# ndoll1998/lightgrad

Measured on AMD Instinct MI355X. Metric: mnist_mlp_train_steps_per_sec_batch1024_per_gpu, higher is better.
Workload: dtype f32; 1 GPU; mnist_mlp_784x512x10_bias_batch1024_mse_adabelief_lr1e-3 (fwd+bwd+allreduce+optimizer); batch_per_gpu=1024, global_batch=1024, parallelism=dp1, optimizer_kernel=fused, input_requires_grad=True, dispatch=hipGraph replay (python tape captured once; 13 consecutive steps per graph), steps_per_graph=13, device=AMD Instinct (gfx950), compute_units=256, clock_mhz=2400

## Files before the change

lightgrad_amd/csrc/gemm.hip:

```cpp
#include "common.h"
#include "gelu_common.h"
#include "adam_common.h"
#include "tail_jobs.h"
#include "mse_finalize.h"
#include "head_fwd_body.h"
#include <cstdlib>
#include <type_traits>

namespace lg {

typedef float f32x16 __attribute__((ext_vector_type(16)));
typedef unsigned int u32x4 __attribute__((ext_vector_type(4)));
typedef float f32x4 __attribute__((ext_vector_type(4)));

#ifndef LG_SMALL_PD
#define LG_SMALL_PD 2
#endif
constexpr int kSmallTilePrefetch = LG_SMALL_PD;

struct FastDiv {
    uint32_t m, s;
    __device__ __forceinline__ int div(int n) const { return int((uint64_t(uint32_t(n)) * m) >> s); }
};
static FastDiv make_fastdiv(int64_t d) {
    if (d < 1) d = 1;
    uint32_t l = 0;
    while ((int64_t(1) << l) < d) ++l;
    FastDiv f;
    f.m = uint32_t((uint64_t(1) << (31 + l)) / uint64_t(d) + 1);
    f.s = 31 + l;
    return f;
}

struct GemmArgs {
    const float* A;
    const float* B;
    float*       C;
    int64_t M, N, K;
    int64_t lda, ldb, ldc;
    int64_t sA, sB, sC;
    int64_t sA2, sB2, sC2;
    int     batch_inner;
    int     tiles_m, tiles_n;
    int     nwg;
    int     accumulate;
    const float* bias;
    const float* addend;
    int64_t      ldadd;
    int     group_m;
    int     k_slices;
    int64_t k_per_slice;
    float*  W;
    int*    tickets;
    float*  rowsum;
    int     rowsum_accumulate;
    FastDiv div_per_batch, div_slices, div_gspan, div_group, div_last_group, div_batch_inner;
    int     k_tail;
    short   relu_a, relu_b;
    int     act;
    float*  aux;
    int     multi;
    int64_t boff[3], coff[3], biasoff[3];
    int     seg_k, seg_steps;
    int64_t seg_jump[2];
    const AdamPlan* adam_c;
    const AdamPlan* adam_r;
#ifdef LG_GEMM_TIMELINE
    unsigned long long* tl;
#endif
};

#ifdef LG_GEMM_TIMELINE
#define LG_TL(slot) do { if (g.tl && threadIdx.x == 0) g.tl[size_t(blockIdx.x) * 8 + (slot)] = wall_clock64(); } while (0)
#else
#define LG_TL(slot) do { } while (0)
#endif

__device__ __forceinline__ int xcd_remap(int bid, int nwg) {
    const int q = nwg >> 3, r = nwg & 7;
    const int xcd = bid & 7, pos = bid >> 3;
    const int base = xcd < r ? xcd * (q + 1) : r * (q + 1) + (xcd - r) * q;
    return base + pos;
}

template <int BM, int BN> constexpr bool kHasExtras = BM * BN < 256 * 256;
template <int BM, int BN, int KG = 1> constexpr bool kCanSplitK = kHasExtras<BM, BN> && KG == 1;
template <int BM, int BN, int KG = 1> constexpr bool kCanAdam = BM * BN <= 128 * 128 && KG == 1;

#ifdef LG_GEMM_GATHER_STAGING
template <int BM, int BN, bool XKC> constexpr bool kGatherStaging = !XKC && BM * BN == 256 * 256;
#else
template <int BM, int BN, bool XKC> constexpr bool kGatherStaging = false;
#endif
template <int BM, int BN, int BK, bool AKC, bool BKC, int KG>
constexpr int gemm_lds_floats() {
    constexpr int BKS = BK * KG;
    constexpr bool ALK = AKC || kGatherStaging<BM, BN, AKC>, BLK = BKC || kGatherStaging<BM, BN, BKC>;
    return 2 * ((ALK ? BM * (BKS + 4) : BKS * BM) + (BLK ? BN * (BKS + 4) : BKS * BN));
}

template <int BM, int BN, int BK, int WM, int WN, bool AKC, bool BKC, bool VA, bool VB, int PD, int KG = 1, int XT = 0>
__global__ void __launch_bounds__(WM * WN * KG * 64) sgemm_mfma(GemmArgs g) {
#define LG_TILE_OWNS_LDS 1
#define LG_TILE_BID blockIdx.x
#include "gemm_tile_body.inc"
#undef LG_TILE_OWNS_LDS
#undef LG_TILE_BID
}

struct HeadChain {
    HeadFwd h;
    int*    tickets;
    int     stride;
    int     per_row;
    int*    status;
};
static const HeadChain*& pending_chain() { static const HeadChain* p = nullptr; return p; }
constexpr int kChainTicketBase = 16384, kChainTicketStride = 32, kChainRowBlocks = 64;
template <int OMAX, int PD>
__global__ void __launch_bounds__(256) sgemm_bias_head_fwd(GemmArgs g, HeadChain c) {
    constexpr int BM = 64, BN = 32, BK = 32, WM = 2, WN = 1, KG = 2, XT = 0;
    constexpr bool AKC = true, BKC = true, VA = true, VB = true;
    __shared__ __attribute__((aligned(16))) float lds[gemm_lds_floats<BM, BN, BK, AKC, BKC, KG>()];
    if (int(blockIdx.x) < g.nwg) {
        int* const signal_tickets = c.tickets;
        const int signal_stride = c.stride, signal_per_row = c.per_row;
#define LG_TILE_OWNS_LDS 0
#define LG_TILE_BID int(blockIdx.x)
#undef LG_TILE_SIGNAL
#define LG_TILE_SIGNAL 1
#include "gemm_tile_body.inc"
#undef LG_TILE_SIGNAL
#undef LG_TILE_BID
#undef LG_TILE_OWNS_LDS
    } else {
        const HeadFwd& a = c.h;
        const int tid = threadIdx.x, lane = tid & 63, wave = tid >> 6;
        const int wn = a.outs * a.hidden;
        for (int i = tid * 4; i < wn; i += 1024) *reinterpret_cast<float4*>(lds + i) = *reinterpret_cast<const float4*>(a.w + i);
        const int64_t row0 = int64_t(int(blockIdx.x) - g.nwg) * 4;
        int* const ticket = c.tickets + int(row0 / BM) * c.stride;
        const int64_t block_rows = a.rows - (row0 / BM) * BM < BM ? a.rows - (row0 / BM) * BM : BM;
        const int readers = int((block_rows + 3) / 4);
        int* const flag = ticket + 16;
        int* const done = ticket + 17;
        __shared__ int seen;
        if (tid == 0) {
            int ok = 1;
            const unsigned long long t0 = wall_clock64();
            while (__hip_atomic_load(flag, __ATOMIC_RELAXED, __HIP_MEMORY_SCOPE_AGENT) == 0) {
                __builtin_amdgcn_s_sleep(2);
                if (wall_clock64() - t0 > 200000000ull) {
                    __hip_atomic_fetch_or(c.status, LG_STATUS_HANDOFF_TIMEOUT, __ATOMIC_RELAXED, __HIP_MEMORY_SCOPE_SYSTEM);
                    ok = 0;
                    break;
                }
            }
            seen = ok;
        }
        __syncthreads();
        __builtin_amdgcn_fence(__ATOMIC_ACQUIRE, "wavefront");
        const int64_t row = row0 + wave;
        if (row < a.rows) head_fwd_row<OMAX, true>(a, lds, row, lane);
        if (tid == 0 && seen) {
            if (__hip_atomic_fetch_add(done, 1, __ATOMIC_RELAXED, __HIP_MEMORY_SCOPE_AGENT) == readers - 1) {
                __hip_atomic_store(done, 0, __ATOMIC_RELAXED, __HIP_MEMORY_SCOPE_AGENT);
                __hip_atomic_store(flag, 0, __ATOMIC_RELAXED, __HIP_MEMORY_SCOPE_AGENT);
            }
        }
    }
}

template <int PD, bool SECOND_BKC = false>
__global__ void __launch_bounds__(256) sgemm_pair_wgrad_xgrad(GemmArgs first, GemmArgs second) {
    constexpr int L1 = gemm_lds_floats<64, 64, 32, false, false, 1>(), L2 = gemm_lds_floats<64, 64, 32, true, SECOND_BKC, 1>();
    __shared__ __attribute__((aligned(16))) float lds[L1 > L2 ? L1 : L2];
    constexpr int BM = 64, BN = 64, BK = 32, WM = 2, WN = 2, KG = 1, XT = 0;
    constexpr bool VA = true, VB = true;
#define LG_TILE_OWNS_LDS 0
    if (int(blockIdx.x) < first.nwg) {
        constexpr bool AKC = false, BKC = false;
        const GemmArgs& g = first;
#define LG_TILE_BID int(blockIdx.x)
#include "gemm_tile_body.inc"
#undef LG_TILE_BID
    } else {
        constexpr bool AKC = true, BKC = SECOND_BKC;
        const GemmArgs& g = second;
#define LG_TILE_BID (int(blockIdx.x) - first.nwg)
#include "gemm_tile_body.inc"
#undef LG_TILE_BID
    }
#undef LG_TILE_OWNS_LDS
}

int lg_mse_finalize_job(const float* row_loss, int64_t rows, float inv_n, float* loss);
struct PairFirsts { GemmArgs w[2]; };
struct LossJob {
    const float* row_loss;
    float*       loss;
    int64_t      rows;
    float        inv_n;
};
template <int PD>
__global__ void __launch_bounds__(256) sgemm_triple_wgrad2_xgrad(PairFirsts firsts, GemmArgs second, LossJob job) {
    constexpr int L1 = gemm_lds_floats<64, 64, 32, false, false, 1>(), L2 = gemm_lds_floats<64, 64, 32, true, false, 1>();
    __shared__ __attribute__((aligned(16))) float lds[L1 > L2 ? L1 : L2];
    constexpr int BM = 64, BN = 64, BK = 32, WM = 2, WN = 2, KG = 1, XT = 0;
    constexpr bool VA = true, VB = true;
#define LG_TILE_OWNS_LDS 0
    const int n0w = firsts.w[0].nwg, n1w = firsts.w[1].nwg;
    if (int(blockIdx.x) < n0w + n1w) {
        constexpr bool AKC = false, BKC = false;
        const int which = int(blockIdx.x) >= n0w ? 1 : 0;
        const GemmArgs g = firsts.w[which];
#define LG_TILE_BID (int(blockIdx.x) - (which ? n0w : 0))
#include "gemm_tile_body.inc"
#undef LG_TILE_BID
    } else if (int(blockIdx.x) < n0w + n1w + second.nwg) {
        constexpr bool AKC = true, BKC = false;
        const GemmArgs& g = second;
#define LG_TILE_BID (int(blockIdx.x) - n0w - n1w)
#include "gemm_tile_body.inc"
#undef LG_TILE_BID
    } else {
        finalize_loss(job.row_loss, job.rows, job.inv_n, job.loss, lds);
    }
#undef LG_TILE_OWNS_LDS
}

constexpr int kGroupMax = 14;
struct GroupProduct {
    const float* A;
    const float* B;
    float*       C;
    float*       W;
    int*         tickets;
    float*       rowsum;
    int64_t      M, N, K, lda, ldb, ldc, k_per_slice;
    int          tiles_m, tiles_n, nwg, accumulate, group_m, k_slices, rowsum_accumulate, k_tail;
    FastDiv      div_per_batch, div_slices, div_gspan, div_group, div_last_group, div_batch_inner;
};
static GroupProduct pack_product(const GemmArgs& g) {
    return GroupProduct{g.A, g.B, g.C, g.W, g.tickets, g.rowsum, g.M, g.N, g.K, g.lda, g.ldb, g.ldc, g.k_per_slice,
                        g.tiles_m, g.tiles_n, g.nwg, g.accumulate, g.group_m, g.k_slices, g.rowsum_accumulate, g.k_tail,
                        g.div_per_batch, g.div_slices, g.div_gspan, g.div_group, g.div_last_group, g.div_batch_inner};
}
__device__ __forceinline__ GemmArgs unpack_product(const GroupProduct& p) {
    GemmArgs g{};
    g.A = p.A; g.B = p.B; g.C = p.C; g.W = p.W; g.tickets = p.tickets; g.rowsum = p.rowsum;
    g.M = p.M; g.N = p.N; g.K = p.K; g.lda = p.lda; g.ldb = p.ldb; g.ldc = p.ldc; g.k_per_slice = p.k_per_slice;
    g.tiles_m = p.tiles_m; g.tiles_n = p.tiles_n; g.nwg = p.nwg; g.accumulate = p.accumulate; g.group_m = p.group_m;
    g.k_slices = p.k_slices; g.rowsum_accumulate = p.rowsum_accumulate; g.k_tail = p.k_tail;
    g.div_per_batch = p.div_per_batch; g.div_slices = p.div_slices; g.div_gspan = p.div_gspan; g.div_group = p.div_group;
    g.div_last_group = p.div_last_group; g.div_batch_inner = p.div_batch_inner;
    g.batch_inner = 1;
    return g;
}

struct GemmGroup {
    GroupProduct p[kGroupMax];
    int      first[kGroupMax + 1];
    int      count;
    const float* cs_in;
    float*       cs_out;
    int64_t      cs_rows, cs_cols, cs_ld;
    int          cs_accumulate, cs_wgs;
    int          tail_wgs;
    TailGroup    tail;
};

static_assert(sizeof(GemmGroup) <= 4096, "the group travels as kernel arguments");

template <int PD>
__global__ void __launch_bounds__(256) sgemm_group_wgrad(GemmGroup grp) {
    __shared__ __attribute__((aligned(16))) float lds[gemm_lds_floats<64, 64, 32, false, false, 1>()];
    constexpr int BM = 64, BN = 64, BK = 32, WM = 2, WN = 2, KG = 1, XT = 0;
    constexpr bool VA = true, VB = true, AKC = false, BKC = false;
    if (int(blockIdx.x) < grp.cs_wgs) {
        const int q = threadIdx.x >> 6, cl = threadIdx.x & 63;
        const int64_t col = int64_t(blockIdx.x) * 64 + cl;
        const bool live = col < grp.cs_cols;
        const float* in = grp.cs_in + (live ? col : 0);
        float acc[8] = {0.f, 0.f, 0.f, 0.f, 0.f, 0.f, 0.f, 0.f};
        int64_t r = q;
        for (; r + 28 < grp.cs_rows; r += 32) {
#pragma unroll
            for (int e = 0; e < 8; ++e) acc[e] += in[(r + 4 * e) * grp.cs_ld];
        }
        for (; r < grp.cs_rows; r += 4) acc[0] += in[r * grp.cs_ld];
        lds[threadIdx.x] = ((acc[0] + acc[1]) + (acc[2] + acc[3])) + ((acc[4] + acc[5]) + (acc[6] + acc[7]));
        __syncthreads();
        if (q == 0 && live) {
            const float v = (lds[cl] + lds[64 + cl]) + (lds[128 + cl] + lds[192 + cl]);
            grp.cs_out[col] = grp.cs_accumulate ? grp.cs_out[col] + v : v;
        }
        return;
    }
    const int bid = int(blockIdx.x) - grp.cs_wgs;
    if (bid >= grp.first[grp.count]) {
        tail_group_body(grp.tail, bid - grp.first[grp.count]);
        return;
    }
    int which = 0;
    while (which + 1 < grp.count && bid >= grp.first[which + 1]) ++which;
    const GemmArgs g = unpack_product(grp.p[which]);
#define LG_TILE_OWNS_LDS 0
#define LG_TILE_BID (bid - grp.first[which])
#include "gemm_tile_body.inc"
#undef LG_TILE_BID
#undef LG_TILE_OWNS_LDS
}

template <int BM, int BN, int BK, int WM, int WN, bool AKC, bool BKC, int KG>
static void launch_layout(const GemmArgs& g, bool va, bool vb) {
    dim3 grid(g.nwg), block(WM * WN * KG * 64);
    hipStream_t s = rt().stream;
    constexpr int PD = (BM * BN <= 64 * 64) ? kSmallTilePrefetch : 2;
    static_assert(BM * BN < 256 * 256 || PD <= 2, "a third K-tile in flight does not fit the 256x256 tile's 128 registers: ring registers would spill while their loads are in flight");
    if constexpr (kHasExtras<BM, BN>) {
        if constexpr (AKC && BKC)  { if (g.multi) { hipLaunchKernelGGL((sgemm_mfma<BM, BN, BK, WM, WN, AKC, BKC, true, true, PD, KG, 1>), grid, block, 0, s, g); return; } }
        if constexpr (AKC && !BKC) { if (g.seg_k) { hipLaunchKernelGGL((sgemm_mfma<BM, BN, BK, WM, WN, AKC, BKC, true, true, PD, KG, 2>), grid, block, 0, s, g); return; } }
    }
    if constexpr (!kHasExtras<BM, BN>) {
        hipLaunchKernelGGL((sgemm_mfma<BM, BN, BK, WM, WN, AKC, BKC, true, true, PD, KG>), grid, block, 0, s, g);
        return;
    }
    if (va && vb)  hipLaunchKernelGGL((sgemm_mfma<BM, BN, BK, WM, WN, AKC, BKC, true, true, PD, KG>), grid, block, 0, s, g);
    else if (va)   hipLaunchKernelGGL((sgemm_mfma<BM, BN, BK, WM, WN, AKC, BKC, true, false, 1, KG>), grid, block, 0, s, g);
    else if (vb)   hipLaunchKernelGGL((sgemm_mfma<BM, BN, BK, WM, WN, AKC, BKC, false, true, 1, KG>), grid, block, 0, s, g);
    else           hipLaunchKernelGGL((sgemm_mfma<BM, BN, BK, WM, WN, AKC, BKC, false, false, 1, KG>), grid, block, 0, s, g);
}

#ifdef LG_GEMM_TIMELINE
static void lg_debug_timeline_state(unsigned long long* buf, int nwg, int slices, int tiles);
#endif
struct PairState {
    int      active = 0;
    int      count = 0;
    bool     second_bkc = false;
    GemmArgs args[3];
    bool     is_s[3] = {false, false, false};
    int64_t  batch[3] = {1, 1, 1};
    int64_t  tiles = 0;
    LossJob  job{};
};
static PairState& pair_state() { static PairState p; return p; }

static void pair_launch_single(const GemmArgs& g, bool is_s) {
    dim3 grid(g.nwg), block(256);
    constexpr int PD = kSmallTilePrefetch;
    if (!is_s) hipLaunchKernelGGL((sgemm_mfma<64, 64, 32, 2, 2, false, false, true, true, PD, 1>), grid, block, 0, rt().stream, g);
    else if (pair_state().second_bkc) hipLaunchKernelGGL((sgemm_mfma<64, 64, 32, 2, 2, true, true, true, true, PD, 1>), grid, block, 0, rt().stream, g);
    else           hipLaunchKernelGGL((sgemm_mfma<64, 64, 32, 2, 2, true, false, true, true, PD, 1>), grid, block, 0, rt().stream, g);
}

static int pair_retune(GemmArgs& g, int64_t others_nwg) {
    const int64_t tiles = int64_t(g.tiles_m) * g.tiles_n;
    static const char* pair_slices_env = getenv("LG_GEMM_PAIR_SLICES");
    if (pair_slices_env || g.nwg != tiles * g.k_slices || g.seg_k || tiles >= 256 || g.K < 128) return LG_OK;
    constexpr int BK = 32, BM = 64, BN = 64;
    const double cus = rt().compute_units > 0 ? rt().compute_units : 256;
    const int64_t k_tiles = (g.K + BK - 1) / BK;
    int64_t best_sl = g.k_slices;
    double best = 1e30;
    for (int64_t sl = 1; sl <= 64 && (sl == 1 || sl * 2 <= k_tiles); ++sl) {
        const double per_cu = double(tiles * sl + others_nwg) / cus;
        const double c = per_cu > 1.0 ? double(int64_t(per_cu + 0.999)) : 1.0;
        const double cost = double((k_tiles + sl - 1) / sl) * (c <= 1.0 ? 0.68 : 0.43 * c + 0.17) + (sl > 1 ? 1.8 + 0.85 * double(sl) : 0.0);
        if (cost < best) { best = cost; best_sl = sl; }
    }
    int64_t k_per_slice = ((g.K + best_sl - 1) / best_sl + BK - 1) / BK * BK;
    best_sl = (g.K + k_per_slice - 1) / k_per_slice;
    if (best_sl == g.k_slices) return LG_OK;
    if (g.W) { const int rc = lg_free(g.W); g.W = nullptr; if (rc != LG_OK) return rc; }
    g.k_per_slice = k_per_slice;
    g.k_slices = int(best_sl);
    g.nwg = int(tiles * best_sl);
    g.div_slices = make_fastdiv(best_sl);
    if (best_sl > 1) {
        const int rc = lg_malloc(reinterpret_cast<void**>(&g.W), size_t(tiles * best_sl) * BM * BN * sizeof(float));
        if (rc != LG_OK) return rc;
    }
    return LG_OK;
}

static int pair_flush(bool keep_collecting) {
    PairState& P = pair_state();
    int rc = LG_OK;
    bool job_done = false;
    if (P.count == 3) {
        rc = pair_retune(P.args[1], int64_t(P.args[0].nwg) + P.args[2].nwg);
        if (rc != LG_OK) { P.count = 0; return rc; }
        PairFirsts firsts;
        firsts.w[0] = P.args[0];
        firsts.w[1] = P.args[1];
        const int spare = P.job.loss ? 1 : 0;
        hipLaunchKernelGGL((sgemm_triple_wgrad2_xgrad<kSmallTilePrefetch>), dim3(P.args[0].nwg + P.args[1].nwg + P.args[2].nwg + spare), dim3(256), 0,
                           rt().stream, firsts, P.args[2], P.job);
        job_done = true;
    } else if (P.count == 2 && P.is_s[1]) {
        rc = pair_retune(P.args[0], P.args[1].nwg);
        if (rc != LG_OK) { P.count = 0; return rc; }
#ifdef LG_GEMM_TIMELINE
        if (P.args[0].tl) {
            (void)hipMemsetAsync(P.args[0].tl, 0, size_t(P.args[0].nwg + P.args[1].nwg) * 64, rt().stream);
            lg_debug_timeline_state(P.args[0].tl, P.args[0].nwg + P.args[1].nwg, P.args[0].k_slices * 100 + P.args[1].k_slices, P.args[0].nwg);
        }
#endif
        if (P.second_bkc)
            hipLaunchKernelGGL((sgemm_pair_wgrad_xgrad<kSmallTilePrefetch, true>), dim3(P.args[0].nwg + P.args[1].nwg), dim3(256), 0, rt().stream,
                               P.args[0], P.args[1]);
        else
            hipLaunchKernelGGL((sgemm_pair_wgrad_xgrad<kSmallTilePrefetch, false>), dim3(P.args[0].nwg + P.args[1].nwg), dim3(256), 0, rt().stream,
                               P.args[0], P.args[1]);
    } else {
        for (int i = 0; i < P.count; ++i) pair_launch_single(P.args[i], P.is_s[i]);
    }
    for (int i = 0; i < P.count; ++i)
        if (P.args[i].W) { const int r = lg_free(P.args[i].W); if (r != LG_OK) rc = r; }
    P.count = 0;
    P.tiles = 0;
    if (job_done) P.job = LossJob{};
    if (!keep_collecting && P.active) P.active = 2;
    return rc;
}

struct WriteSpan { uintptr_t lo, hi; };
static WriteSpan product_c_span(const GemmArgs& g, int64_t batch) {
    const int64_t outer = batch / g.batch_inner;
    int64_t lo = 0, hi = (g.M - 1) * g.ldc + g.N;
    const int64_t reach[2] = {(outer - 1) * g.sC, int64_t(g.batch_inner - 1) * g.sC2};
    for (int64_t r : reach) { if (r < 0) lo += r; else hi += r; }
    const uintptr_t base = reinterpret_cast<uintptr_t>(g.C);
    return WriteSpan{base + uintptr_t(lo * 4), base + uintptr_t(hi * 4)};
}
static bool spans_meet(WriteSpan a, WriteSpan b) { return a.lo < b.hi && b.lo < a.hi; }
static bool products_write_alike(const GemmArgs& a, int64_t batch_a, const GemmArgs& b, int64_t batch_b) {
    const WriteSpan none{0, 0};
    const WriteSpan ca = product_c_span(a, batch_a), cb = product_c_span(b, batch_b);
    const WriteSpan ra = a.rowsum ? WriteSpan{reinterpret_cast<uintptr_t>(a.rowsum), reinterpret_cast<uintptr_t>(a.rowsum + a.M)} : none;
    const WriteSpan rb = b.rowsum ? WriteSpan{reinterpret_cast<uintptr_t>(b.rowsum), reinterpret_cast<uintptr_t>(b.rowsum + b.M)} : none;
    return spans_meet(ca, cb) || spans_meet(ca, rb) || spans_meet(ra, cb) || spans_meet(ra, rb);
}

static bool pair_try_defer(GemmArgs& g, bool akc, bool bkc, bool va, bool vb, int64_t batch) {
    PairState& P = pair_state();
    if (P.active != 1) return false;
    const int slot = P.count;
    for (int i = 0; i < slot; ++i)
        if (products_write_alike(P.args[i], P.batch[i], g, batch)) return false;
    const bool f_form = !akc && !bkc, s_form = akc;
    bool fits = slot < 3 && va && vb && batch >= 1;
    if (slot == 0)      fits = fits && f_form;
    else if (slot == 1) fits = fits && !P.is_s[0] && (f_form || s_form);
    else                fits = fits && !P.is_s[1] && s_form && !bkc && batch == 1 && !g.relu_a && !g.relu_b;
    if (slot == 1 && f_form) fits = fits && batch == 1 && P.args[0].nwg == int64_t(P.args[0].tiles_m) * P.args[0].tiles_n * P.args[0].k_slices;
    const int64_t tiles = int64_t(g.tiles_m) * g.tiles_n * batch;
    if (!fits || P.tiles + tiles > rt().n_gemm_tickets) return false;
    g.tickets = rt().gemm_tickets + P.tiles;
    P.tiles += tiles;
    if (s_form) P.second_bkc = bkc;
    P.is_s[slot] = s_form;
    P.args[slot] = g;
    P.batch[slot] = batch;
    P.count = slot + 1;
    return true;
}

constexpr int kGroupTiles = 1024;
struct GroupState {
    int       active = 0;
// ... 577 lines not shown
```

lightgrad_amd/csrc/gemm_tile_body.inc:

```
#ifndef LG_TILE_SIGNAL
#define LG_TILE_SIGNAL 0
#endif
    constexpr int NT = WM * WN * KG * 64;
    constexpr int BKS = BK * KG;
    constexpr int TM = BM / WM / 32, TN = BN / WN / 32;
    static_assert(TM >= 1 && TN >= 1 && BK % 16 == 0 && (KG == 1 || KG == 2 || KG == 4), "tile config");
    constexpr bool AG = kGatherStaging<BM, BN, AKC>, BG = kGatherStaging<BM, BN, BKC>;
    static_assert((!AG || VA) && (!BG || VB), "gather staging replaces the float4 form");
    constexpr bool ALK = AKC || AG, BLK = BKC || BG;
    constexpr int A_PITCH = ALK ? BKS + 4 : BM;
    constexpr int B_PITCH = BLK ? BKS + 4 : BN;
    constexpr int A_TILE = ALK ? BM * A_PITCH : BKS * A_PITCH;
    constexpr int B_TILE = BLK ? BN * B_PITCH : BKS * B_PITCH;
    constexpr int A_ELEMS = BM * BKS / NT, B_ELEMS = BN * BKS / NT;
    static_assert(A_ELEMS % 4 == 0 && B_ELEMS % 4 == 0, "staging must divide into float4");

    static_assert(2 * (A_TILE + B_TILE) == gemm_lds_floats<BM, BN, BK, AKC, BKC, KG>(), "LDS size");
    static_assert(!(AG || BG) || TM * TN > 1, "gather staging: the multi-accumulator loop only");
#if LG_TILE_OWNS_LDS
    __shared__ __attribute__((aligned(16))) float lds[2 * (A_TILE + B_TILE)];
#endif
    constexpr int BUF = A_TILE + B_TILE;

    const int tid = threadIdx.x;
    const int lane = tid & 63, wave = tid >> 6;
    const int kg = wave / (WM * WN), wl = wave % (WM * WN);
    const int wm = wl / WN, wn = wl % WN;
    const int kofs = kg * BK;
    const int r = lane & 31, h = lane >> 5;
    LG_TL(0);

    const int id = xcd_remap(LG_TILE_BID, g.nwg);
    const int per_batch = g.tiles_m * g.tiles_n;
    const int bs = g.div_per_batch.div(id);
    const int batch = g.div_slices.div(bs), slice = bs - batch * g.k_slices;
    const int t = id - bs * per_batch;
    const int GROUP_M = g.group_m;
    const int gspan = GROUP_M * g.tiles_n;
    const int group = g.div_gspan.div(t);
    const int first_m = group * GROUP_M, in_group = t - group * gspan;
    const bool last_group = g.tiles_m - first_m < GROUP_M;
    const int gsize = last_group ? g.tiles_m - first_m : GROUP_M;
    const int tn = last_group ? g.div_last_group.div(in_group) : g.div_group.div(in_group);
    const int tm = first_m + (in_group - tn * gsize);
    const int64_t m0 = int64_t(tm) * BM, n0 = int64_t(tn) * BN;
    const int b_outer = g.div_batch_inner.div(batch), b_inner = batch - b_outer * g.batch_inner;
    const float* __restrict__ A = g.A + int64_t(b_outer) * g.sA + int64_t(b_inner) * g.sA2;
    const float* Bp = g.B + int64_t(b_outer) * g.sB + int64_t(b_inner) * g.sB2;
    float* Cp = g.C + int64_t(b_outer) * g.sC + int64_t(b_inner) * g.sC2;
    const float* biasp = g.bias;
    if constexpr (XT == 1) {
        {
            Bp += batch == 0 ? g.boff[0] : batch == 1 ? g.boff[1] : g.boff[2];
            Cp += batch == 0 ? g.coff[0] : batch == 1 ? g.coff[1] : g.coff[2];
            if (biasp) biasp += batch == 0 ? g.biasoff[0] : batch == 1 ? g.biasoff[1] : g.biasoff[2];
        }
    }
    const float* __restrict__ B = Bp;
    float* __restrict__ C = Cp;
    const int64_t ldc = g.ldc;
    const int accumulate = g.accumulate;
    const float* __restrict__ bias = biasp;
    const int64_t k_begin = int64_t(slice) * g.k_per_slice;
    const int64_t k_end = (k_begin + g.k_per_slice < g.K) ? k_begin + g.k_per_slice : g.K;
    const bool has_virtual = kHasExtras<BM, BN> && g.rowsum != nullptr && n0 <= g.N && g.N < n0 + BN;

    using StageA = std::conditional_t<VA, f32x4, float>;
    using StageB = std::conditional_t<VB, f32x4, float>;
    constexpr int A_CHUNKS = VA ? A_ELEMS / 4 : A_ELEMS, B_CHUNKS = VB ? B_ELEMS / 4 : B_ELEMS;
    constexpr int NL = (kGatherStaging<BM, BN, AKC> ? 4 : 1) * A_CHUNKS + (kGatherStaging<BM, BN, BKC> ? 4 : 1) * B_CHUNKS;
    static_assert((PD - 1) * NL + NL <= 63, "vmcnt is a 6-bit counter");
    StageA ra_ring[PD][A_CHUNKS];
    StageB rb_ring[PD][B_CHUNKS];
    [[maybe_unused]] float ga_ring[PD][AG ? A_CHUNKS : 1][4];
    [[maybe_unused]] float gb_ring[PD][BG ? B_CHUNKS : 1][4];

    constexpr unsigned OOB = 0x80000000u;
    constexpr int A_W = VA ? 4 : 1, B_W = VB ? 4 : 1;
    constexpr int A_DIV = AG ? BM : (AKC ? BKS : BM) / A_W, B_DIV = BG ? BN : (BKC ? BKS : BN) / B_W;
    static_assert(NT % A_DIV == 0 && NT % B_DIV == 0, "a thread's chunks must differ by whole rows");
    constexpr int A_STEP = NT / A_DIV, B_STEP = NT / B_DIV;
    const int a_q = tid / A_DIV, a_r = AG ? tid % A_DIV : (tid % A_DIV) * A_W;
    const int b_q = tid / B_DIV, b_r = BG ? tid % B_DIV : (tid % B_DIV) * B_W;
    auto kcA = [&](int i) { return AG ? 4 * (a_q + i * A_STEP) : (AKC ? a_r : a_q + i * A_STEP); };
    auto kcB = [&](int i) { return BG ? 4 * (b_q + i * B_STEP) : (BKC ? b_r : b_q + i * B_STEP); };
    const int a_lds0 = AG ? a_r * A_PITCH + 4 * a_q : a_q * A_PITCH + a_r, b_lds0 = BG ? b_r * B_PITCH + 4 * b_q : b_q * B_PITCH + b_r;
    constexpr int A_LDS_STEP = AG ? 4 * A_STEP : A_STEP * A_PITCH, B_LDS_STEP = BG ? 4 * B_STEP : B_STEP * B_PITCH;
    unsigned offA[A_CHUNKS], offB[B_CHUNKS];
    unsigned virt_mask = 0;
    int krem_ring[PD];
#pragma unroll
    for (int i = 0; i < A_CHUNKS; ++i) {
        const int row = AKC ? a_q + i * A_STEP : a_r, kk = kcA(i);
        const unsigned bytes = AKC ? (unsigned(row) * unsigned(g.lda) + unsigned(kk)) * 4u : (unsigned(kk) * unsigned(g.lda) + unsigned(row)) * 4u;
        offA[i] = (m0 + row < g.M) ? bytes : OOB;
    }
#pragma unroll
    for (int i = 0; i < B_CHUNKS; ++i) {
        const int col = BKC ? b_q + i * B_STEP : b_r, kk = kcB(i);
        const unsigned bytes = BKC ? (unsigned(col) * unsigned(g.ldb) + unsigned(kk)) * 4u : (unsigned(kk) * unsigned(g.ldb) + unsigned(col)) * 4u;
        offB[i] = (n0 + col < g.N) ? bytes : OOB;
        if (has_virtual && n0 + col == g.N) virt_mask |= 1u << i;
    }
    const float* const Atile0 = AKC ? A + m0 * g.lda : A + m0;
    const float* const Btile0 = BKC ? B + n0 * g.ldb : B + n0;

    auto descriptor = [](const float* base) {
        const unsigned long long p = reinterpret_cast<unsigned long long>(base);
        u32x4 d;
        d[0] = unsigned(p); d[1] = unsigned(p >> 32) & 0xffffu; d[2] = OOB; d[3] = 0x00020000u;
        return d;
    };
    const float* nextA = AKC ? Atile0 + k_begin : Atile0 + k_begin * g.lda;
    const float* nextB = BKC ? Btile0 + k_begin : Btile0 + k_begin * g.ldb;
    const int64_t stepA = AKC ? int64_t(BKS) : int64_t(BKS) * g.lda, stepB = BKC ? int64_t(BKS) : int64_t(BKS) * g.ldb;
    [[maybe_unused]] const unsigned gatherA = unsigned(g.lda) * 4u, gatherB = unsigned(g.ldb) * 4u;
    const int nkt = int((k_end - k_begin + BKS - 1) / BKS);
    const int last_krem = int(k_end - k_begin) - (nkt - 1) * BKS;
    int requested = 0;
    int seg_left = 0, seg_idx = 0;
    if constexpr (XT == 2) seg_left = g.seg_steps;
    auto load_tile = [&](int slot) {
        const int krem = requested == nkt - 1 ? last_krem : BKS;
        ++requested;
        krem_ring[slot] = krem;
        const u32x4 da = descriptor(nextA);
        const u32x4 db = descriptor(nextB);
        nextA += stepA;
        nextB += stepB;
        if constexpr (XT == 2) {
            if (--seg_left == 0) {
                nextB += seg_idx ? g.seg_jump[1] : g.seg_jump[0];
                seg_idx = 1;
                seg_left = g.seg_steps;
            }
        }
#pragma unroll
        for (int i = 0; i < A_CHUNKS; ++i) {
            if constexpr (AG) {
                if (krem == BKS) {
#pragma unroll
                    for (int e = 0; e < 4; ++e)
                        asm volatile("buffer_load_dword %0, %1, %2, %3 offen" : "=v"(ga_ring[slot][i][e]) : "v"(offA[i]), "s"(da), "s"(unsigned(e) * gatherA));
                } else {
#pragma unroll
                    for (int e = 0; e < 4; ++e) {
                        const unsigned off = kcA(i) + e < krem ? offA[i] : OOB;
                        asm volatile("buffer_load_dword %0, %1, %2, %3 offen" : "=v"(ga_ring[slot][i][e]) : "v"(off), "s"(da), "s"(unsigned(e) * gatherA));
                    }
                }
            } else {
                const unsigned off = kcA(i) < krem ? offA[i] : OOB;
                if constexpr (VA) asm volatile("buffer_load_dwordx4 %0, %1, %2, 0 offen" : "=v"(ra_ring[slot][i]) : "v"(off), "s"(da));
                else              asm volatile("buffer_load_dword %0, %1, %2, 0 offen" : "=v"(ra_ring[slot][i]) : "v"(off), "s"(da));
            }
        }
#pragma unroll
        for (int i = 0; i < B_CHUNKS; ++i) {
            if constexpr (BG) {
                if (krem == BKS) {
#pragma unroll
                    for (int e = 0; e < 4; ++e)
                        asm volatile("buffer_load_dword %0, %1, %2, %3 offen" : "=v"(gb_ring[slot][i][e]) : "v"(offB[i]), "s"(db), "s"(unsigned(e) * gatherB));
                } else {
#pragma unroll
                    for (int e = 0; e < 4; ++e) {
                        const unsigned off = kcB(i) + e < krem ? offB[i] : OOB;
                        asm volatile("buffer_load_dword %0, %1, %2, %3 offen" : "=v"(gb_ring[slot][i][e]) : "v"(off), "s"(db), "s"(unsigned(e) * gatherB));
                    }
                }
            } else {
                const unsigned off = kcB(i) < krem ? offB[i] : OOB;
                if constexpr (VB) asm volatile("buffer_load_dwordx4 %0, %1, %2, 0 offen" : "=v"(rb_ring[slot][i]) : "v"(off), "s"(db));
                else              asm volatile("buffer_load_dword %0, %1, %2, 0 offen" : "=v"(rb_ring[slot][i]) : "v"(off), "s"(db));
            }
        }
    };
    auto wait_tile = [&](int slot, int younger) {
        if (PD >= 3 && younger >= 2)      asm volatile("s_waitcnt vmcnt(%0)" :: "n"(PD >= 3 ? 2 * NL : 0) : "memory");
        else if (PD >= 2 && younger == 1) asm volatile("s_waitcnt vmcnt(%0)" :: "n"(PD >= 2 ? NL : 0) : "memory");
        else                              asm volatile("s_waitcnt vmcnt(0)" ::: "memory");
#pragma unroll
        for (int i = 0; i < A_CHUNKS; ++i) {
            if constexpr (AG) { asm volatile("" : "+v"(ga_ring[slot][i][0]), "+v"(ga_ring[slot][i][1]), "+v"(ga_ring[slot][i][2]), "+v"(ga_ring[slot][i][3])); }
            else              asm volatile("" : "+v"(ra_ring[slot][i]));
        }
#pragma unroll
        for (int i = 0; i < B_CHUNKS; ++i) {
            if constexpr (BG) { asm volatile("" : "+v"(gb_ring[slot][i][0]), "+v"(gb_ring[slot][i][1]), "+v"(gb_ring[slot][i][2]), "+v"(gb_ring[slot][i][3])); }
            else              asm volatile("" : "+v"(rb_ring[slot][i]));
        }
    };

    auto store_tile = [&](int buf, int slot) {
        float* a = lds + buf * BUF;
        float* b = lds + buf * BUF + A_TILE;
        if (g.k_tail && krem_ring[slot] < BKS) {
            asm volatile("; short K tail" ::: "memory");
            if constexpr (VA && AKC) {
#pragma unroll
                for (int i = 0; i < A_CHUNKS; ++i)
#pragma unroll
                    for (int e = 1; e < 4; ++e)
                        if (kcA(i) + e >= krem_ring[slot]) ra_ring[slot][i][e] = 0.f;
            }
            if constexpr (VB && BKC) {
#pragma unroll
                for (int i = 0; i < B_CHUNKS; ++i)
#pragma unroll
                    for (int e = 1; e < 4; ++e)
                        if (kcB(i) + e >= krem_ring[slot]) rb_ring[slot][i][e] = 0.f;
            }
        }
        if constexpr (kHasExtras<BM, BN>) if (g.relu_a) {
            asm volatile("; relu(A) on the way to LDS" ::: "memory");
#pragma unroll
            for (int i = 0; i < A_CHUNKS; ++i) {
                if constexpr (VA) {
#pragma unroll
                    for (int e = 0; e < 4; ++e) { const float x = ra_ring[slot][i][e]; ra_ring[slot][i][e] = (x != x) ? x : (x > 0.0f ? x : 0.0f); }
                } else {
                    const float x = ra_ring[slot][i]; ra_ring[slot][i] = (x != x) ? x : (x > 0.0f ? x : 0.0f);
                }
            }
        }
#pragma unroll
        for (int i = 0; i < A_CHUNKS; ++i) {
            if constexpr (AG)      *reinterpret_cast<f32x4*>(a + a_lds0 + i * A_LDS_STEP) = f32x4{ga_ring[slot][i][0], ga_ring[slot][i][1], ga_ring[slot][i][2], ga_ring[slot][i][3]};
            else if constexpr (VA) *reinterpret_cast<f32x4*>(a + a_lds0 + i * A_LDS_STEP) = ra_ring[slot][i];
            else                   a[a_lds0 + i * A_LDS_STEP] = ra_ring[slot][i];
        }
        if constexpr (kHasExtras<BM, BN>) if (g.relu_b) {
            asm volatile("; relu(B) on the way to LDS" ::: "memory");
#pragma unroll
            for (int i = 0; i < B_CHUNKS; ++i) {
                if constexpr (VB) {
#pragma unroll
                    for (int e = 0; e < 4; ++e) { const float x = rb_ring[slot][i][e]; rb_ring[slot][i][e] = (x != x) ? x : (x > 0.0f ? x : 0.0f); }
                } else {
                    const float x = rb_ring[slot][i]; rb_ring[slot][i] = (x != x) ? x : (x > 0.0f ? x : 0.0f);
                }
            }
        }
        if constexpr (kHasExtras<BM, BN>) if (has_virtual) {
#pragma unroll
            for (int i = 0; i < B_CHUNKS; ++i) {
                const bool virt = (virt_mask >> i) & 1u, kv = kcB(i) < krem_ring[slot];
                const float one = kv ? 1.0f : 0.0f;
                if constexpr (VB) {
                    if constexpr (BKC) {
                        if (virt) {
                            const int kr = krem_ring[slot] - kcB(i);
                            rb_ring[slot][i] = f32x4{kr > 0 ? 1.f : 0.f, kr > 1 ? 1.f : 0.f, kr > 2 ? 1.f : 0.f, kr > 3 ? 1.f : 0.f};
                        }
                    }
                    else               { if (virt) rb_ring[slot][i] = f32x4{one, 0.f, 0.f, 0.f}; }
                } else {
                    if (virt) rb_ring[slot][i] = one;
                }
            }
        }
#pragma unroll
        for (int i = 0; i < B_CHUNKS; ++i) {
            if constexpr (BG)      *reinterpret_cast<f32x4*>(b + b_lds0 + i * B_LDS_STEP) = f32x4{gb_ring[slot][i][0], gb_ring[slot][i][1], gb_ring[slot][i][2], gb_ring[slot][i][3]};
            else if constexpr (VB) *reinterpret_cast<f32x4*>(b + b_lds0 + i * B_LDS_STEP) = rb_ring[slot][i];
            else                   b[b_lds0 + i * B_LDS_STEP] = rb_ring[slot][i];
        }
    };

    f32x16 acc[TM][TN];
    [[maybe_unused]] float bias_ahead[TN];
    if constexpr (kHasExtras<BM, BN>) {
#pragma unroll
        for (int j = 0; j < TN; ++j) {
            const int64_t col = n0 + (wn * TN + j) * 32 + r;
            bias_ahead[j] = (bias && col < g.N) ? bias[col] : 0.f;
        }
    }
#pragma unroll
    for (int i = 0; i < TM; ++i)
#pragma unroll
        for (int j = 0; j < TN; ++j)
#pragma unroll
            for (int e = 0; e < 16; ++e) acc[i][j][e] = 0.f;

    auto compute_tile = [&](int buf, int kb_begin, int kb_end) {
        const float* a = lds + buf * BUF + (ALK ? (wm * TM * 32 + r) * A_PITCH + 4 * h + kofs : (4 * h + kofs) * A_PITCH + wm * TM * 32 + r);
        const float* b = lds + buf * BUF + A_TILE + (BLK ? (wn * TN * 32 + r) * B_PITCH + 4 * h + kofs : (4 * h + kofs) * B_PITCH + wn * TN * 32 + r);
#pragma unroll
        for (int kb = kb_begin; kb < kb_end; kb += 8) {
            float fa[TM][4], fb[TN][4];
#pragma unroll
            for (int i = 0; i < TM; ++i) {
                if constexpr (ALK) {
                    const float4 v = *reinterpret_cast<const float4*>(a + i * 32 * A_PITCH + kb);
                    fa[i][0] = v.x; fa[i][1] = v.y; fa[i][2] = v.z; fa[i][3] = v.w;
                } else {
#pragma unroll
                    for (int s = 0; s < 4; ++s) fa[i][s] = a[(kb + s) * A_PITCH + i * 32];
                }
            }
#pragma unroll
            for (int j = 0; j < TN; ++j) {
                if constexpr (BLK) {
                    const float4 v = *reinterpret_cast<const float4*>(b + j * 32 * B_PITCH + kb);
                    fb[j][0] = v.x; fb[j][1] = v.y; fb[j][2] = v.z; fb[j][3] = v.w;
                } else {
#pragma unroll
                    for (int s = 0; s < 4; ++s) fb[j][s] = b[(kb + s) * B_PITCH + j * 32];
                }
            }
#pragma unroll
            for (int s = 0; s < 4; ++s)
#pragma unroll
                for (int i = 0; i < TM; ++i)
#pragma unroll
                    for (int j = 0; j < TN; ++j)
                        acc[i][j] = __builtin_amdgcn_mfma_f32_32x32x2f32(fa[i][s], fb[j][s], acc[i][j], 0, 0, 0);
        }
    };

#pragma unroll
    for (int u = 0; u < PD; ++u)
        if (u < nkt) load_tile(u);
    {
        const int younger = nkt - 1 < PD - 1 ? nkt - 1 : PD - 1;
        wait_tile(0, younger);
    }
    store_tile(0, 0);
    __syncthreads();
    LG_TL(1);
    if constexpr (TM * TN == 1) {
        constexpr int HG = BK / 16;
        float fa[2][HG][4], fb[2][HG][4];
        auto read_half = [&](int buf, int half, int slot) {
            const float* a = lds + buf * BUF + (AKC ? (wm * 32 + r) * A_PITCH + 4 * h + kofs : (4 * h + kofs) * A_PITCH + wm * 32 + r);
            const float* b = lds + buf * BUF + A_TILE + (BKC ? (wn * 32 + r) * B_PITCH + 4 * h + kofs : (4 * h + kofs) * B_PITCH + wn * 32 + r);
#pragma unroll
            for (int q = 0; q < HG; ++q) {
                const int kb = half * (BK / 2) + q * 8;
                if constexpr (AKC) {
                    const float4 v = *reinterpret_cast<const float4*>(a + kb);
                    fa[slot][q][0] = v.x; fa[slot][q][1] = v.y; fa[slot][q][2] = v.z; fa[slot][q][3] = v.w;
                } else {
#pragma unroll
                    for (int e = 0; e < 4; ++e) fa[slot][q][e] = a[(kb + e) * A_PITCH];
                }
                if constexpr (BKC) {
                    const float4 v = *reinterpret_cast<const float4*>(b + kb);
                    fb[slot][q][0] = v.x; fb[slot][q][1] = v.y; fb[slot][q][2] = v.z; fb[slot][q][3] = v.w;
                } else {
#pragma unroll
                    for (int e = 0; e < 4; ++e) fb[slot][q][e] = b[(kb + e) * B_PITCH];
                }
            }
        };
        auto mfma_part = [&](int slot, int q0, int q1) {
#pragma unroll
            for (int q = q0; q < q1; ++q)
#pragma unroll
                for (int e = 0; e < 4; ++e)
                    acc[0][0] = __builtin_amdgcn_mfma_f32_32x32x2f32(fa[slot][q][e], fb[slot][q][e], acc[0][0], 0, 0, 0);
        };
        auto mfma_half = [&](int slot) { mfma_part(slot, 0, HG); };
        constexpr int HQ = HG > 1 ? HG / 2 : HG;
        read_half(0, 0, 0);
        for (int kt0 = 0; kt0 < nkt; kt0 += PD) {
#pragma unroll
            for (int u = 0; u < PD; ++u) {
                const int kt = kt0 + u;
                if (kt < nkt) {
                    const int cur = kt & 1;
                    if (PD == 1 && kt + 1 < nkt) load_tile(0);
                    read_half(cur, 1, 1);
                    mfma_part(0, 0, HQ);
                    __builtin_amdgcn_sched_barrier(0);
                    if (kt + 1 < nkt) {
                        int younger = nkt - (kt + 2);
                        if (younger > PD - 2) younger = PD - 2;
                        wait_tile((u + 1) % PD, PD == 1 ? 0 : (younger < 0 ? 0 : younger));
                        store_tile(cur ^ 1, (u + 1) % PD);
                    }
                    if (PD > 1 && kt + PD < nkt) load_tile(u);
                    __builtin_amdgcn_sched_barrier(0);
                    mfma_part(0, HQ, HG);
                    __syncthreads();
                    if (kt + 1 < nkt) read_half(cur ^ 1, 0, 0);
                    mfma_half(1);
                }
            }
        }
    } else {
        for (int kt0 = 0; kt0 < nkt; kt0 += PD) {
    #pragma unroll
            for (int u = 0; u < PD; ++u) {
                const int kt = kt0 + u;
                if (kt < nkt) {
                    const int cur = kt & 1;
                    if (PD == 1 && kt + 1 < nkt) load_tile(0);
                    compute_tile(cur, 0, BK / 2);
                    if (kt + 1 < nkt) {
                        int younger = nkt - (kt + 2);
                        if (younger > PD - 2) younger = PD - 2;
                        wait_tile((u + 1) % PD, PD == 1 ? 0 : (younger < 0 ? 0 : younger));
                        store_tile(cur ^ 1, (u + 1) % PD);
                    }
                    if (PD > 1 && kt + PD < nkt) load_tile(u);
                    compute_tile(cur, BK / 2, BK);
                    __syncthreads();
                }
            }
        }
    }

    LG_TL(2);
    if constexpr (KG > 1) {
        constexpr int GROUP_FLOATS = WM * WN * TM * TN * 16 * 64;
        static_assert((KG - 1) * GROUP_FLOATS <= 2 * (A_TILE + B_TILE), "the K-group exchange must fit the staging buffers");
        float* x = lds + (wl * TM * TN * 16) * 64 + lane;
        if (kg >= 1) {
#pragma unroll
            for (int i = 0; i < TM; ++i)
#pragma unroll
                for (int j = 0; j < TN; ++j)
#pragma unroll
                    for (int e = 0; e < 16; ++e) x[(kg - 1) * GROUP_FLOATS + ((i * TN + j) * 16 + e) * 64] = acc[i][j][e];
        }
        __syncthreads();
        if (kg >= 1) return;
#pragma unroll
        for (int gq = 0; gq < KG - 1; ++gq)
#pragma unroll
            for (int i = 0; i < TM; ++i)
#pragma unroll
                for (int j = 0; j < TN; ++j)
#pragma unroll
                    for (int e = 0; e < 16; ++e) acc[i][j][e] += x[gq * GROUP_FLOATS + ((i * TN + j) * 16 + e) * 64];
    }
    [[maybe_unused]] AdamScalars adam_cs_c, adam_cs_r;
    [[maybe_unused]] int64_t adam_done_c = 0, adam_done_r = 0;
    if constexpr (kCanAdam<BM, BN, KG>) {
        if (g.adam_c) adam_cs_c = adam_plan_scalars(g.adam_c, adam_done_c);
        if (g.adam_r) adam_cs_r = adam_plan_scalars(g.adam_r, adam_done_r);
    }
    if constexpr (kCanSplitK<BM, BN, KG>) if (g.k_slices > 1) {
        constexpr int SC1 = 16;
        constexpr int TILE_BYTES = BM * BN * 4;
        char* slab0 = reinterpret_cast<char*>(g.W) + (int64_t(batch) * g.k_slices * per_batch + t) * int64_t(TILE_BYTES);
        const int64_t slice_stride = int64_t(per_batch) * TILE_BYTES;
        {
            const auto mine = __builtin_amdgcn_make_buffer_rsrc(slab0 + slice * slice_stride, 0, TILE_BYTES, 0x00020000);
#pragma unroll
            for (int i = 0; i < TM; ++i)
#pragma unroll
                for (int j = 0; j < TN; ++j)
#pragma unroll
                    for (int q = 0; q < 4; ++q) {
                        u32x4 v;
#pragma unroll
                        for (int e = 0; e < 4; ++e) v[e] = __float_as_uint(acc[i][j][4 * q + e]);
                        __builtin_amdgcn_raw_buffer_store_b128(v, mine, (((i * TN + j) * 4 + q) * NT + tid) * 16, 0, SC1);
                    }
        }
        asm volatile("s_waitcnt vmcnt(0)" ::: "memory");
        __syncthreads();
        LG_TL(3);
        int* arrived_last = reinterpret_cast<int*>(lds);
        if (tid == 0) {
            int* ticket = g.tickets + batch * per_batch + t;
            const int order = __hip_atomic_fetch_add(ticket, 1, __ATOMIC_RELAXED, __HIP_MEMORY_SCOPE_AGENT);
            const int last = order == g.k_slices - 1;
            if (last) __hip_atomic_store(ticket, 0, __ATOMIC_RELAXED, __HIP_MEMORY_SCOPE_AGENT);
            *arrived_last = last;
        }
        __syncthreads();
        LG_TL(4);
        if (!*arrived_last) return;
        __builtin_amdgcn_fence(__ATOMIC_ACQUIRE, "wavefront");
        constexpr int CH = TM * TN >= 4 ? 1 : (TM * TN == 2 ? 2 : 4);
        for (int s0 = 0; s0 < g.k_slices; s0 += CH) {
            u32x4 v[CH][TM * TN * 4];
#pragma unroll
            for (int c = 0; c < CH; ++c) {
                const int sl = s0 + c < g.k_slices ? s0 + c : s0;
                const auto src = __builtin_amdgcn_make_buffer_rsrc(slab0 + sl * slice_stride, 0, TILE_BYTES, 0x00020000);
#pragma unroll
                for (int f = 0; f < TM * TN * 4; ++f) v[c][f] = __builtin_amdgcn_raw_buffer_load_b128(src, (f * NT + tid) * 16, 0, SC1);
            }
#pragma unroll
            for (int c = 0; c < CH; ++c) {
                const bool live = s0 + c < g.k_slices, first = s0 + c == 0;
#pragma unroll
                for (int i = 0; i < TM; ++i)
#pragma unroll
                    for (int j = 0; j < TN; ++j)
#pragma unroll
                        for (int e = 0; e < 16; ++e) {
                            const float w = __uint_as_float(v[c][(i * TN + j) * 4 + e / 4][e % 4]);
                            acc[i][j][e] = first ? w : (live ? acc[i][j][e] + w : acc[i][j][e]);
                        }
            }
        }
    }

    LG_TL(5);
    int etid = threadIdx.x;
    asm volatile("" : "+v"(etid));
    const int ewl = (etid >> 6) % (WM * WN), er = etid & 31, eh = (etid >> 5) & 1;
    const int ewm = ewl / WN, ewn = ewl % WN;
#pragma unroll
    for (int i = 0; i < TM; ++i) {
#pragma unroll
        for (int j = 0; j < TN; ++j) {
            const int64_t col = n0 + (ewn * TN + j) * 32 + er;
            const int64_t row0 = m0 + (ewm * TM + i) * 32 + 4 * eh;
            const bool vcol = has_virtual && col == g.N;
            if (col < g.N || vcol) {
                float bv = 0.f;
                if constexpr (kHasExtras<BM, BN>) bv = (bias && !vcol) ? bias_ahead[j] : 0.f;
                else                              bv = bias ? bias[col] : 0.f;
                float* const dst = vcol ? g.rowsum : C + col;
                const int64_t dstride = vcol ? 1 : ldc;
                const float* const addend = vcol ? nullptr : g.addend;
                const bool acc_flag = vcol ? g.rowsum_accumulate != 0 : (accumulate != 0 || addend != nullptr);
                const float* const old_src = addend ? addend + col : dst;
                const int64_t old_stride = addend ? g.ldadd : dstride;
                float val[16];
#pragma unroll
                for (int e = 0; e < 16; ++e) val[e] = bias ? acc[i][j][e] + bv : acc[i][j][e];
                if (acc_flag) {
                    float old[16];
#pragma unroll
                    for (int e = 0; e < 16; ++e) {
                        const int64_t row = row0 + (e & 3) + 8 * (e >> 2);
                        old[e] = row < g.M ? old_src[row * old_stride] : 0.f;
                    }
#pragma unroll
                    for (int e = 0; e < 16; ++e) val[e] = old[e] + val[e];
                }
                if constexpr (kHasExtras<BM, BN>) {
                    if (g.act == 2 && !vcol) {
                        float x[16];
#pragma unroll
                        for (int e = 0; e < 16; ++e) {
                            const int64_t row = row0 + (e & 3) + 8 * (e >> 2);
                            x[e] = row < g.M ? g.aux[row * g.ldadd + col] : 0.f;
                        }
#pragma unroll
                        for (int e = 0; e < 16; ++e) val[e] = gelu_grad(x[e], val[e]);
                    }
                }
                float* p = dst + row0 * dstride;
#pragma unroll
                for (int e = 0; e < 16; ++e) {
                    const int64_t row = row0 + (e & 3) + 8 * (e >> 2);
#if LG_TILE_SIGNAL
                    if (row < g.M) __hip_atomic_store(p + ((e & 3) + 8 * (e >> 2)) * dstride, val[e], __ATOMIC_RELAXED, __HIP_MEMORY_SCOPE_AGENT);
#else
                    if (row < g.M) p[((e & 3) + 8 * (e >> 2)) * dstride] = val[e];
#endif
                }
                if constexpr (kCanAdam<BM, BN, KG>) {
                    const AdamPlan* const pl = vcol ? g.adam_r : g.adam_c;
                    if (pl) {
                        const AdamScalars& cs = vcol ? adam_cs_r : adam_cs_c;
                        const int64_t base = vcol ? row0 : row0 * ldc + col;
                        const float* const pin = pl->p_in + base;
                        float* const pout = pl->p_out + base;
                        float* const pm = pl->m + base;
                        float* const pv = pl->v + base;
#pragma unroll
                        for (int half = 0; half < 2; ++half) {
// ... 56 lines not shown
```

Before: 20460 steps/s.

## Add wave-private K loop for 32x32 K-grouped GEMM tiles without block barriers

For 32x32 tiles that use one wave per K-group, each wave now stages its own interleaved K-slices into a private LDS region. It runs its own software-pipelined load/store/MFMA loop with no __syncthreads in the main loop, and the per-wave partial sums are reduced through an exchange region at the end. This is meant to remove block-wide barrier stalls and cross-wave coupling in the small-tile GEMMs. It adds a separate code path with single-buffered staging per wave (default prefetch depth 1), which may expose load latency. The old cooperative loop can be selected with an environment variable.

Result: faster. 21190 steps/s (median of 6 runs) (+3.6%).

```diff
diff --git a/lightgrad_amd/csrc/gemm.hip b/lightgrad_amd/csrc/gemm.hip
--- a/lightgrad_amd/csrc/gemm.hip
+++ b/lightgrad_amd/csrc/gemm.hip
@@ -5,6 +5,7 @@
 #include "mse_finalize.h"
 #include "head_fwd_body.h"
 #include <cstdlib>
+#include <cstring>
 #include <type_traits>
 
 namespace lg {
@@ -17,6 +18,10 @@
 #define LG_SMALL_PD 2
 #endif
 constexpr int kSmallTilePrefetch = LG_SMALL_PD;
+#ifndef LG_WAVE_PRIVATE_PD
+#define LG_WAVE_PRIVATE_PD 1
+#endif
+constexpr int kWavePrivatePrefetch = LG_WAVE_PRIVATE_PD;
 
 struct FastDiv {
     uint32_t m, s;
@@ -92,6 +97,7 @@
 #else
 template <int BM, int BN, bool XKC> constexpr bool kGatherStaging = false;
 #endif
+template <int BM, int BN, int WM, int WN, int KG> constexpr bool kWavePrivateTile = KG > 1 && WM * WN == 1 && BM == 32 && BN == 32;
 template <int BM, int BN, int BK, bool AKC, bool BKC, int KG>
 constexpr int gemm_lds_floats() {
     constexpr int BKS = BK * KG;
@@ -99,11 +105,13 @@
     return 2 * ((ALK ? BM * (BKS + 4) : BKS * BM) + (BLK ? BN * (BKS + 4) : BKS * BN));
 }
 
-template <int BM, int BN, int BK, int WM, int WN, bool AKC, bool BKC, bool VA, bool VB, int PD, int KG = 1, int XT = 0>
+template <int BM, int BN, int BK, int WM, int WN, bool AKC, bool BKC, bool VA, bool VB, int PD, int KG = 1, int XT = 0, bool WP = false>
 __global__ void __launch_bounds__(WM * WN * KG * 64) sgemm_mfma(GemmArgs g) {
 #define LG_TILE_OWNS_LDS 1
 #define LG_TILE_BID blockIdx.x
+#define LG_TILE_WAVE_PRIVATE WP
 #include "gemm_tile_body.inc"
+#undef LG_TILE_WAVE_PRIVATE
 #undef LG_TILE_OWNS_LDS
 #undef LG_TILE_BID
 }
@@ -318,6 +326,15 @@
     hipStream_t s = rt().stream;
     constexpr int PD = (BM * BN <= 64 * 64) ? kSmallTilePrefetch : 2;
     static_assert(BM * BN < 256 * 256 || PD <= 2, "a third K-tile in flight does not fit the 256x256 tile's 128 registers: ring registers would spill while their loads are in flight");
+    if constexpr (kWavePrivateTile<BM, BN, WM, WN, KG> && AKC && BKC) {
+        static const char* kloop_env = getenv("LG_GEMM_KLOOP");
+        if (va && vb && !(kloop_env && strcmp(kloop_env, "coop") == 0)) {
+            constexpr int WPD = kWavePrivatePrefetch;
+            if (g.multi) hipLaunchKernelGGL((sgemm_mfma<BM, BN, BK, WM, WN, true, true, true, true, WPD, KG, 1, true>), grid, block, 0, s, g);
+            else         hipLaunchKernelGGL((sgemm_mfma<BM, BN, BK, WM, WN, true, true, true, true, WPD, KG, 0, true>), grid, block, 0, s, g);
+            return;
+        }
+    }
     if constexpr (kHasExtras<BM, BN>) {
         if constexpr (AKC && BKC)  { if (g.multi) { hipLaunchKernelGGL((sgemm_mfma<BM, BN, BK, WM, WN, AKC, BKC, true, true, PD, KG, 1>), grid, block, 0, s, g); return; } }
         if constexpr (AKC && !BKC) { if (g.seg_k) { hipLaunchKernelGGL((sgemm_mfma<BM, BN, BK, WM, WN, AKC, BKC, true, true, PD, KG, 2>), grid, block, 0, s, g); return; } }
diff --git a/lightgrad_amd/csrc/gemm_tile_body.inc b/lightgrad_amd/csrc/gemm_tile_body.inc
--- a/lightgrad_amd/csrc/gemm_tile_body.inc
+++ b/lightgrad_amd/csrc/gemm_tile_body.inc
@@ -1,8 +1,14 @@
 #ifndef LG_TILE_SIGNAL
 #define LG_TILE_SIGNAL 0
 #endif
+#ifndef LG_TILE_WAVE_PRIVATE
+#define LG_TILE_WAVE_PRIVATE false
+#endif
+    constexpr bool WPK = LG_TILE_WAVE_PRIVATE;
+    static_assert(!WPK || (KG > 1 && WM * WN == 1 && BM == 32 && BN == 32 && AKC && BKC && VA && VB && XT != 2 && !LG_TILE_SIGNAL), "wave-private K loop: one wave per K-group, NT form");
     constexpr int NT = WM * WN * KG * 64;
-    constexpr int BKS = BK * KG;
+    constexpr int NTS = WPK ? 64 : NT;
+    constexpr int BKS = WPK ? BK : BK * KG;
     constexpr int TM = BM / WM / 32, TN = BN / WN / 32;
     static_assert(TM >= 1 && TN >= 1 && BK % 16 == 0 && (KG == 1 || KG == 2 || KG == 4), "tile config");
     constexpr bool AG = kGatherStaging<BM, BN, AKC>, BG = kGatherStaging<BM, BN, BKC>;
@@ -12,21 +18,23 @@
     constexpr int B_PITCH = BLK ? BKS + 4 : BN;
     constexpr int A_TILE = ALK ? BM * A_PITCH : BKS * A_PITCH;
     constexpr int B_TILE = BLK ? BN * B_PITCH : BKS * B_PITCH;
-    constexpr int A_ELEMS = BM * BKS / NT, B_ELEMS = BN * BKS / NT;
+    constexpr int A_ELEMS = BM * BKS / NTS, B_ELEMS = BN * BKS / NTS;
     static_assert(A_ELEMS % 4 == 0 && B_ELEMS % 4 == 0, "staging must divide into float4");
 
-    static_assert(2 * (A_TILE + B_TILE) == gemm_lds_floats<BM, BN, BK, AKC, BKC, KG>(), "LDS size");
+    static_assert(WPK || 2 * (A_TILE + B_TILE) == gemm_lds_floats<BM, BN, BK, AKC, BKC, KG>(), "LDS size");
     static_assert(!(AG || BG) || TM * TN > 1, "gather staging: the multi-accumulator loop only");
 #if LG_TILE_OWNS_LDS
-    __shared__ __attribute__((aligned(16))) float lds[2 * (A_TILE + B_TILE)];
+    __shared__ __attribute__((aligned(16))) float lds[gemm_lds_floats<BM, BN, BK, AKC, BKC, KG>()];
 #endif
     constexpr int BUF = A_TILE + B_TILE;
 
     const int tid = threadIdx.x;
     const int lane = tid & 63, wave = tid >> 6;
-    const int kg = wave / (WM * WN), wl = wave % (WM * WN);
+    const int kg = WPK ? __builtin_amdgcn_readfirstlane(wave) : wave / (WM * WN), wl = wave % (WM * WN);
     const int wm = wl / WN, wn = wl % WN;
-    const int kofs = kg * BK;
+    const int kofs = WPK ? 0 : kg * BK;
+    const int stid = WPK ? lane : tid;
+    float* const ldsw = WPK ? lds + kg * BUF : lds;
     const int r = lane & 31, h = lane >> 5;
     LG_TL(0);
 
@@ -78,10 +86,10 @@
     constexpr unsigned OOB = 0x80000000u;
     constexpr int A_W = VA ? 4 : 1, B_W = VB ? 4 : 1;
     constexpr int A_DIV = AG ? BM : (AKC ? BKS : BM) / A_W, B_DIV = BG ? BN : (BKC ? BKS : BN) / B_W;
-    static_assert(NT % A_DIV == 0 && NT % B_DIV == 0, "a thread's chunks must differ by whole rows");
-    constexpr int A_STEP = NT / A_DIV, B_STEP = NT / B_DIV;
-    const int a_q = tid / A_DIV, a_r = AG ? tid % A_DIV : (tid % A_DIV) * A_W;
-    const int b_q = tid / B_DIV, b_r = BG ? tid % B_DIV : (tid % B_DIV) * B_W;
+    static_assert(NTS % A_DIV == 0 && NTS % B_DIV == 0, "a thread's chunks must differ by whole rows");
+    constexpr int A_STEP = NTS / A_DIV, B_STEP = NTS / B_DIV;
+    const int a_q = stid / A_DIV, a_r = AG ? stid % A_DIV : (stid % A_DIV) * A_W;
+    const int b_q = stid / B_DIV, b_r = BG ? stid % B_DIV : (stid % B_DIV) * B_W;
     auto kcA = [&](int i) { return AG ? 4 * (a_q + i * A_STEP) : (AKC ? a_r : a_q + i * A_STEP); };
     auto kcB = [&](int i) { return BG ? 4 * (b_q + i * B_STEP) : (BKC ? b_r : b_q + i * B_STEP); };
     const int a_lds0 = AG ? a_r * A_PITCH + 4 * a_q : a_q * A_PITCH + a_r, b_lds0 = BG ? b_r * B_PITCH + 4 * b_q : b_q * B_PITCH + b_r;
@@ -111,12 +119,20 @@
         d[0] = unsigned(p); d[1] = unsigned(p >> 32) & 0xffffu; d[2] = OOB; d[3] = 0x00020000u;
         return d;
     };
-    const float* nextA = AKC ? Atile0 + k_begin : Atile0 + k_begin * g.lda;
-    const float* nextB = BKC ? Btile0 + k_begin : Btile0 + k_begin * g.ldb;
-    const int64_t stepA = AKC ? int64_t(BKS) : int64_t(BKS) * g.lda, stepB = BKC ? int64_t(BKS) : int64_t(BKS) * g.ldb;
+    constexpr int KSTEP = BK * KG;
+    int64_t wk_begin = k_begin, wk_len = k_end - k_begin;
+    if constexpr (WPK) {
+        wk_begin = k_begin + kg * BK;
+        wk_len = wk_len - kg * BK;
+        wk_len = wk_len < 0 ? 0 : wk_len;
+    }
+    const float* nextA = AKC ? Atile0 + wk_begin : Atile0 + wk_begin * g.lda;
+    const float* nextB = BKC ? Btile0 + wk_begin : Btile0 + wk_begin * g.ldb;
+    const int64_t stepA = AKC ? int64_t(KSTEP) : int64_t(KSTEP) * g.lda, stepB = BKC ? int64_t(KSTEP) : int64_t(KSTEP) * g.ldb;
     [[maybe_unused]] const unsigned gatherA = unsigned(g.lda) * 4u, gatherB = unsigned(g.ldb) * 4u;
-    const int nkt = int((k_end - k_begin + BKS - 1) / BKS);
-    const int last_krem = int(k_end - k_begin) - (nkt - 1) * BKS;
+    const int nkt = int((wk_len + KSTEP - 1) / KSTEP);
+    const int last_left = int(wk_len) - (nkt - 1) * KSTEP;
+    const int last_krem = last_left < BKS ? last_left : BKS;
     int requested = 0;
     int seg_left = 0, seg_idx = 0;
     if constexpr (XT == 2) seg_left = g.seg_steps;
@@ -193,8 +209,8 @@
     };
 
     auto store_tile = [&](int buf, int slot) {
-        float* a = lds + buf * BUF;
-        float* b = lds + buf * BUF + A_TILE;
+        float* a = ldsw + buf * BUF;
+        float* b = ldsw + buf * BUF + A_TILE;
         if (g.k_tail && krem_ring[slot] < BKS) {
             asm volatile("; short K tail" ::: "memory");
             if constexpr (VA && AKC) {
@@ -323,14 +339,55 @@
 #pragma unroll
     for (int u = 0; u < PD; ++u)
         if (u < nkt) load_tile(u);
-    {
+    if constexpr (!WPK) {
         const int younger = nkt - 1 < PD - 1 ? nkt - 1 : PD - 1;
         wait_tile(0, younger);
-    }
-    store_tile(0, 0);
-    __syncthreads();
+        store_tile(0, 0);
+        __syncthreads();
+    }
     LG_TL(1);
-    if constexpr (TM * TN == 1) {
+    if constexpr (WPK) {
+        static_assert(BK == 16, "one K-step is two k-blocks of 8");
+        float fa[2][4], fb[2][4];
+        auto read_half = [&](int half, int set) {
+            const float4 va = *reinterpret_cast<const float4*>(ldsw + r * A_PITCH + 4 * h + half * 8);
+            const float4 vb = *reinterpret_cast<const float4*>(ldsw + A_TILE + r * B_PITCH + 4 * h + half * 8);
+            fa[set][0] = va.x; fa[set][1] = va.y; fa[set][2] = va.z; fa[set][3] = va.w;
+            fb[set][0] = vb.x; fb[set][1] = vb.y; fb[set][2] = vb.z; fb[set][3] = vb.w;
+        };
+        auto mfma_part = [&](int set, int e0, int e1) {
+#pragma unroll
+            for (int e = e0; e < e1; ++e)
+                acc[0][0] = __builtin_amdgcn_mfma_f32_32x32x2f32(fa[set][e], fb[set][e], acc[0][0], 0, 0, 0);
+        };
+        auto advance = [&](int t, int slot) {
+            const int younger = (nkt < t + PD ? nkt : t + PD) - (t + 1);
+            wait_tile(slot, younger);
+            store_tile(0, slot);
+            if (t + PD < nkt) load_tile(slot);
+        };
+        if (nkt > 0) {
+            advance(0, 0);
+            read_half(0, 0);
+        }
+        for (int kt0 = 0; kt0 < nkt; kt0 += PD) {
+#pragma unroll
+            for (int u = 0; u < PD; ++u) {
+                const int kt = kt0 + u;
+                if (kt < nkt) {
+                    read_half(1, 1);
+                    mfma_part(0, 0, 4);
+                    __builtin_amdgcn_sched_barrier(0);
+                    if (kt + 1 < nkt) advance(kt + 1, (u + 1) % PD);
+                    __builtin_amdgcn_sched_barrier(0);
+                    mfma_part(1, 0, 1);
+                    __builtin_amdgcn_sched_barrier(0);
+                    if (kt + 1 < nkt) read_half(0, 0);
+                    mfma_part(1, 1, 4);
+                }
+            }
+        }
+    } else if constexpr (TM * TN == 1) {
         constexpr int HG = BK / 16;
         float fa[2][HG][4], fb[2][HG][4];
         auto read_half = [&](int buf, int half, int slot) {
@@ -416,8 +473,9 @@
     LG_TL(2);
     if constexpr (KG > 1) {
         constexpr int GROUP_FLOATS = WM * WN * TM * TN * 16 * 64;
-        static_assert((KG - 1) * GROUP_FLOATS <= 2 * (A_TILE + B_TILE), "the K-group exchange must fit the staging buffers");
-        float* x = lds + (wl * TM * TN * 16) * 64 + lane;
+        static_assert(WPK || (KG - 1) * GROUP_FLOATS <= 2 * (A_TILE + B_TILE), "the K-group exchange must fit the staging buffers");
+        static_assert(!WPK || KG * BUF + (KG - 1) * GROUP_FLOATS <= gemm_lds_floats<BM, BN, BK, AKC, BKC, KG>(), "staging regions + exchange");
+        float* x = lds + (WPK ? KG * BUF : 0) + (wl * TM * TN * 16) * 64 + lane;
         if (kg >= 1) {
 #pragma unroll
             for (int i = 0; i < TM; ++i)
```
